# kohnakagawa/md_neighbor_list

Hardware: AMD Instinct MI355X
Metric: Verlet-list build ms and Mpairs/s at N=1M rho=1.0; achieved HBM GB/s (higher is better)
Workload: dtype f32

## Files before the change

md_neighbor_list_amd/csrc/nl_kernels.hpp:

```cpp
#pragma once

#include <hip/hip_runtime.h>
#include <stdint.h>

#include <type_traits>

namespace nl {

constexpr int WAVE = 64;

enum : uint32_t { ST_OUT_OF_BOX = 1u, ST_CAPACITY = 2u, ST_DOMAIN = 4u, ST_INDEX_OVERFLOW = 8u, ST_ROW_OVERFLOW = 16u };

template <typename T> struct Pos;
template <> struct alignas(16) Pos<float> {
  float x, y, z;
  int32_t gid;
};
template <> struct alignas(32) Pos<double> {
  double x, y, z;
  int32_t gid;
  int32_t row;
};

struct Box {
// ... 675 lines not shown
    const T t = mul_rn(q, ims);
    const T f = sub_rn(t, (T)(int32_t)t);
    return (f >= (T)0.25 ? 1 : 0) + (f >= (T)0.5 ? 1 : 0) + (f >= (T)0.75 ? 1 : 0);
  };
  const bool tilt = !FINE && IDC == 0 && g.tilt;
  auto bin_of = [&](const Pos<T>& p) {
    const int32_t c = tilt ? p.gid : xcell1(p.x);
    if constexpr (FINE) return quarter(p.z, g.ims[2]) * mx + c;
    else if constexpr (IDC > 0) return c * IDC + min((int32_t)((uint32_t)p.gid >> id_shift), IDC - 1);
    else return c;
  };
  constexpr int BC_KEEP = 6;
  const bool keep = end - beg <= BC_KEEP * 256 && end > beg && !(g.dbg & 512);
  Pos<T> pk[BC_KEEP];
  int32_t rk[BC_KEEP];
  if (keep) {
#pragma unroll
    for (int u = 0; u < BC_KEEP; u++) {
      const int32_t k = min(beg + tid + u * 256, end - 1);
      pk[u] = src[k];
      rk[u] = src_row[k];
    }
#pragma unroll
    for (int u = 0; u < BC_KEEP; u++) {
      keep_in_flight(pk[u].x), keep_in_flight(pk[u].y), keep_in_flight(pk[u].z), keep_in_flight(pk[u].gid), keep_in_flight(rk[u]);
      if constexpr (sizeof(T) == 8) keep_in_flight(pk[u].row);
    }
#pragma unroll
    for (int u = 0; u < BC_KEEP; u++)
      if (beg + tid + u * 256 < end) atomicAdd(&cnt[bin_of(pk[u])], 1);
  } else {
    for (int32_t k = beg + tid; k < end; k += 256) atomicAdd(&cnt[bin_of(src[k])], 1);
  }
  __syncthreads();
  for (int32_t base = 0; base < nb; base += 256) {
    const int32_t c = base + tid;
    const int32_t v = c < nb ? cnt[c] : 0;
    const int32_t inc = wave_incl_scan(v, lane);
    if (lane == 63) wsum[w] = inc;
    __syncthreads();
    int32_t woff = 0;
    for (int k = 0; k < w; k++) woff += wsum[k];
    const int32_t carry = carry_s;
    const int32_t excl = carry + woff + inc - v;
    if (c < nb) {
      cnt[c] = excl;
      if constexpr (FINE) {
        cell_start[((size_t)r * mx + (c % mx)) * 4 + c / mx] = beg + excl;
      } else if constexpr (IDC > 0) {
        cls_start[(size_t)r * nb + c] = beg + excl;
        if (c % IDC == 0) cell_start[(size_t)r * mx + c / IDC] = beg + excl;
      } else {
        cell_start[(size_t)r * nb + c] = beg + excl;
      }
    }
    __syncthreads();
    if (tid == 255) carry_s = carry + woff + inc;
    __syncthreads();
  }
  if (r == nrows - 1 && tid == 0) {
    if constexpr (IDC > 0) cls_start[(size_t)nrows * nb] = end, cell_start[(size_t)nrows * mx] = end;
    else cell_start[(size_t)nrows * nb] = end;
  }
  auto place = [&](Pos<T> p, int32_t row_of) {
    const int32_t dst = beg + atomicAdd(&cnt[bin_of(p)], 1);
    if (tilt) {
      p.gid = row_of;
    } else if (g.pbc & 1) {
      const T tx = mul_rn(p.x, g.ims[0]);
      int32_t v = (int32_t)tx;
      if (tx < (T)0 && (T)v != tx) v -= 1;
      if (v < 0) p.x = add_rn(p.x, g.L[0]);
      if (v >= mx) p.x = add_rn(p.x, -g.L[0]);
    }
    sorted[dst] = p;
    sorted_row[dst] = row_of;
    sorted_gid[dst] = p.gid;
  };
  if (keep) {
#pragma unroll
    for (int u = 0; u < BC_KEEP; u++)
      if (beg + tid + u * 256 < end) place(pk[u], rk[u]);
  } else {
    for (int32_t k = beg + tid; k < end; k += 256) place(src[k], src_row[k]);
  }
}

enum { MODE_COUNT = 0, MODE_FILL = 1, MODE_COUNT_MASKS = 2 };

struct FastDiv {
  uint32_t d, m, s;
};
__device__ __forceinline__ uint32_t fastdiv(uint32_t n, const FastDiv& f) {
  if (f.d == 1) return n;
  const uint32_t t = __umulhi(n, f.m);
  return (t + ((n - t) >> 1)) >> (f.s - 1);
}

template <typename T> struct SweepArgs {
  const Pos<T>* __restrict__ sorted;
  const int32_t* __restrict__ sorted_row;
  const int32_t* __restrict__ sorted_gid;
  const int32_t* __restrict__ cell_start;
  const int32_t* __restrict__ cls_start;
  int32_t mx, my, mzl, slab;
  FastDiv div_mx, div_my;
  T rc2;
  int32_t* __restrict__ count;
  int32_t* __restrict__ progress;
  const void* __restrict__ key_pointer;
  int32_t wide;
  int32_t n_rows;
  int32_t* __restrict__ list;
  const int64_t* __restrict__ total;
  int64_t capacity;
  uint32_t* __restrict__ status;
  T L[3];
  int32_t pbc;
  T ms[3];
  int32_t z_origin;
  int32_t isplit;
  int32_t mask_nb;
  int32_t* __restrict__ full27_list;
  int32_t* __restrict__ full27_count;
  int32_t* __restrict__ fill_list_count;
  uint32_t* __restrict__ masks;
  uint8_t* __restrict__ masks_hi;
  unsigned long long* dbg_buf;
  int32_t dbg;
  const uint32_t* gate = nullptr;
  T k[3];
  const double* lat;
};

template <typename T>
__device__ __forceinline__ void face_shift(const SweepArgs<T>& a, int32_t wr, T& sx, T& sy, T& sz) {
  T s[3];
  lattice_shift(a.lat, wr, s);
  sx = s[0], sy = s[1], sz = s[2];
}

__device__ __forceinline__ void recheck_image(const SweepArgs<double>& a, int32_t wr, Pos<double>& pe) {
  const double* p = a.lat + 3 * wr;
  pe.x = add_rn(pe.x, p[0]);
  __builtin_amdgcn_sched_barrier(0);
  pe.y = add_rn(pe.y, p[1]);
  __builtin_amdgcn_sched_barrier(0);
  pe.z = add_rn(pe.z, p[2]);
}

template <typename T> struct SweepCfg;
constexpr int MASK_LO_BYTES = 2 * WAVE, MASK_HI_BYTES = WAVE, MASK_ROW_BYTES = MASK_LO_BYTES + MASK_HI_BYTES;
__device__ __forceinline__ bool hi_plane_used(int32_t mask_nb, int32_t ntiles) { return mask_nb > 1 || ntiles > 16; }
template <bool NT = false>
__device__ __forceinline__ void mask_store(uint32_t* masks, uint8_t* masks_hi, size_t row, int lane, uint32_t bits, bool hi) {
  uint16_t* const lo_p = reinterpret_cast<uint16_t*>(reinterpret_cast<char*>(masks) + row * MASK_LO_BYTES) + lane;
  uint8_t* const hi_p = masks_hi + row * MASK_HI_BYTES + lane;
  if constexpr (NT) {
    __builtin_nontemporal_store((uint16_t)bits, lo_p);
    if (hi) __builtin_nontemporal_store((uint8_t)(bits >> 16), hi_p);
  } else {
    *lo_p = (uint16_t)bits;
    if (hi) *hi_p = (uint8_t)(bits >> 16);
  }
}
template <bool NT, typename P> __device__ __forceinline__ P mask_ld(const P* p) {
  if constexpr (NT) return __builtin_nontemporal_load(p);
  else return *p;
}
__device__ __forceinline__ uint32_t mask_load(const uint32_t* masks, const uint8_t* masks_hi, size_t row, int lane) {
  return (uint32_t)reinterpret_cast<const uint16_t*>(reinterpret_cast<const char*>(masks) + row * MASK_LO_BYTES)[lane] |
         (uint32_t)(masks_hi + row * MASK_HI_BYTES)[lane] << 16;
}
template <> struct SweepCfg<float> { static constexpr int CAP = 1280; };
template <> struct SweepCfg<double> { static constexpr int CAP = 1280; };

constexpr int SWEEP_WAVES = 4;
constexpr int SWEEP_G = 5;
constexpr int NSEG = 18;

struct alignas(16) PosS {
  float x, y, z;
  int32_t gid;
};
struct ScreenCtx {
  float lo, hi;
  float lo_in, hi_out;
  const int32_t* sidx;
  const uint8_t* swrap;
};
template <typename T, bool SCREEN> struct TileOf { typedef Pos<T> type; };
template <typename T> struct TileOf<T, true> { typedef PosS type; };

#ifndef NL_STAMP
#define NL_STAMP 0
#endif
#ifndef NL_STAMP_FILL
#define NL_STAMP_FILL 0
#endif
#ifndef NL_DIAG
#define NL_DIAG 0
#endif
constexpr int NL_PRIO = 3;
template <int GC>
__device__ __forceinline__ void r2_group_f32(float xj, float yj, float zj, const float* xi, const float* yi, const float* zi, float* r2) {
#pragma unroll
  for (int k = 0; k < GC; k++) {
    const float dx = sub_rn(xj, xi[k]), dy = sub_rn(yj, yi[k]), dz = sub_rn(zj, zi[k]);
    r2[k] = add_rn(add_rn(mul_rn(dx, dx), mul_rn(dy, dy)), mul_rn(dz, dz));
  }
}

template <typename T, int MODE, int GC, bool FULL = false, bool NOSELF = false, bool SCREEN = false, bool PBC = false>
__device__ __forceinline__ int32_t search_group(const SweepArgs<T>& a, const typename TileOf<T, SCREEN>::type* tile, int32_t nj,
                                                int32_t ntiles, int lane, const Pos<T>& pi_l, int64_t base_l,
                                                int32_t slot0 = 0, bool store_masks = false, int32_t self0 = 0, int32_t batch = 0,
                                                const ScreenCtx* sc = nullptr, float uxi_l = 0.f, float uyi_l = 0.f, float uzi_l = 0.f,
                                                uint32_t* words_out = nullptr) {
  static_assert(!NOSELF || (FULL && MODE == MODE_COUNT_MASKS), "NOSELF is a form of the full-list COUNT_MASKS search");
  static_assert(SweepCfg<T>::CAP / WAVE <= 24, "one bit per j-tile in the 24-bit word a lane keeps (mask_store)");
  static_assert(!SCREEN || sizeof(T) == 8, "the screened search is the fp64 search");
  typedef typename TileOf<T, SCREEN>::type TileT;
  typedef typename std::conditional<SCREEN, float, T>::type R;
  R xi[GC], yi[GC], zi[GC];
  int32_t gi[GC];
  uint32_t cur[GC];
  int32_t* rowp[GC];
  uint32_t bits[GC];
  constexpr bool VBITS_F32 = MODE == MODE_COUNT_MASKS && !SCREEN && sizeof(T) == 4 && (!FULL || NOSELF);
  constexpr bool VBITS_SCREEN = MODE == MODE_COUNT_MASKS && SCREEN && (!FULL || NOSELF);
  constexpr bool VBITS = VBITS_F32 || VBITS_SCREEN;
  uint32_t gi1[GC];
#pragma unroll
  for (int k = 0; k < GC; k++) bits[k] = 0;
#pragma unroll
  for (int k = 0; k < GC; k++) {
    if constexpr (SCREEN) {
      xi[k] = __builtin_bit_cast(float, __builtin_amdgcn_readlane(__builtin_bit_cast(int32_t, uxi_l), k));
      yi[k] = __builtin_bit_cast(float, __builtin_amdgcn_readlane(__builtin_bit_cast(int32_t, uyi_l), k));
      zi[k] = __builtin_bit_cast(float, __builtin_amdgcn_readlane(__builtin_bit_cast(int32_t, uzi_l), k));
    } else if constexpr (sizeof(T) == 4) {
      xi[k] = __builtin_bit_cast(float, __builtin_amdgcn_readlane(__builtin_bit_cast(int32_t, pi_l.x), k));
      yi[k] = __builtin_bit_cast(float, __builtin_amdgcn_readlane(__builtin_bit_cast(int32_t, pi_l.y), k));
      zi[k] = __builtin_bit_cast(float, __builtin_amdgcn_readlane(__builtin_bit_cast(int32_t, pi_l.z), k));
    } else {
      xi[k] = __shfl(pi_l.x, k, WAVE);
      yi[k] = __shfl(pi_l.y, k, WAVE);
      zi[k] = __shfl(pi_l.z, k, WAVE);
    }
    gi[k] = __builtin_amdgcn_readlane(pi_l.gid, k);
    cur[k] = 0u;
    gi1[k] = (uint32_t)gi[k] + 1u;
    if (MODE == MODE_FILL) {
      const uint32_t lo = (uint32_t)__builtin_amdgcn_readlane((int32_t)(uint32_t)base_l, k);
      const uint32_t hi = (uint32_t)__builtin_amdgcn_readlane((int32_t)(uint32_t)((uint64_t)base_l >> 32), k);
      rowp[k] = a.list + (int64_t)(((uint64_t)hi << 32) | lo);
    }
  }

  auto test_tile = [&](const TileT& pj, int32_t tix) {
    if constexpr (VBITS_SCREEN) {
      constexpr int HALF = (GC + 1) / 2;
      uint32_t uacc = 0;
#pragma unroll
      for (int k = 0; k < GC; k++) {
        if (k == HALF) __builtin_amdgcn_sched_barrier(0);
        const float dx = pj.x - xi[k], dy = pj.y - yi[k], dz = pj.z - zi[k];
        const float r2 = __builtin_fmaf(dz, dz, __builtin_fmaf(dy, dy, dx * dx));
        const uint32_t t_in = __builtin_bit_cast(uint32_t, sc->lo_in - r2), t_out = __builtin_bit_cast(uint32_t, r2 - sc->hi_out);
        uint32_t w = t_in;
        if (!NOSELF) w |= (uint32_t)pj.gid - gi1[k];
        bits[k] = __builtin_amdgcn_alignbit(bits[k], w, 31);
        uacc |= t_in & t_out;
      }
      if (__builtin_amdgcn_ballot_w64((int32_t)uacc < 0) != 0) {
        const int32_t at = tix * WAVE + lane;
        Pos<double> pe;
        pe.x = 0, pe.y = 0, pe.z = 0;
        if ((int32_t)uacc < 0) {
          pe = a.sorted[sc->sidx[at]];
          if (PBC) recheck_image(a, sc->swrap[at], pe);
        }
#pragma unroll
        for (int k = 0; k < GC; k++) {
          const float dx = pj.x - xi[k], dy = pj.y - yi[k], dz = pj.z - zi[k];
          const float r2 = __builtin_fmaf(dz, dz, __builtin_fmaf(dy, dy, dx * dx));
          const bool unc = (int32_t)(__builtin_bit_cast(uint32_t, sc->lo_in - r2) & __builtin_bit_cast(uint32_t, r2 - sc->hi_out)) < 0;
          if (__builtin_amdgcn_ballot_w64(unc) == 0) continue;
          const double xe = __hiloint2double(__builtin_amdgcn_readlane(__double2hiint(pi_l.x), k), __builtin_amdgcn_readlane(__double2loint(pi_l.x), k));
          const double ye = __hiloint2double(__builtin_amdgcn_readlane(__double2hiint(pi_l.y), k), __builtin_amdgcn_readlane(__double2loint(pi_l.y), k));
          const double ze = __hiloint2double(__builtin_amdgcn_readlane(__double2hiint(pi_l.z), k), __builtin_amdgcn_readlane(__double2loint(pi_l.z), k));
          const double ex = sub_rn(pe.x, xe), ey = sub_rn(pe.y, ye), ez = sub_rn(pe.z, ze);
          const double e2 = add_rn(add_rn(mul_rn(ex, ex), mul_rn(ey, ey)), mul_rn(ez, ez));
          const bool upper = NOSELF ? true : pj.gid > gi[k];
          if (unc && !(e2 > a.rc2) && upper) bits[k] &= ~1u;
        }
      }
      return;
    }
    if constexpr (VBITS_F32) {
      constexpr int HALF = (GC + 1) / 2;
#pragma unroll
      for (int k = 0; k < GC; k++) {
        if (k == HALF) __builtin_amdgcn_sched_barrier(0);
        const float dx = sub_rn(pj.x, xi[k]), dy = sub_rn(pj.y, yi[k]), dz = sub_rn(pj.z, zi[k]);
        const float r2 = add_rn(add_rn(mul_rn(dx, dx), mul_rn(dy, dy)), mul_rn(dz, dz));
// ... 453 lines not shown
  }
#endif
}

template <typename T, int MODE> constexpr int sweep_cap() { return SweepCfg<T>::CAP; }

template <typename T, int MODE, bool FULL = false, bool PBC = false>
__device__ __forceinline__ void sweep_cell(const SweepArgs<T>& a) {
  if (gate_closed(a.gate)) return;
  constexpr int CAP = sweep_cap<T, MODE>();
  constexpr bool SCREEN = sizeof(T) == 8;
  __shared__ __attribute__((aligned(32))) char tile_bytes[SCREEN ? screen_lds_bytes(CAP) : CAP * (int)sizeof(Pos<T>)];
  Pos<T>* const tile = reinterpret_cast<Pos<T>*>(tile_bytes);
  if (MODE == MODE_FILL) {
    if (a.total[0] > a.capacity) {
      if (blockIdx.x == 0 && threadIdx.x == 0) atomicOr(a.status, ST_CAPACITY);
      return;
    }
  }
  const int tid = threadIdx.x, lane = tid & 63, wave = __builtin_amdgcn_readfirstlane(tid >> 6);
  CellCtx c;
  if (MODE == MODE_COUNT_MASKS) __builtin_amdgcn_s_setprio(NL_PRIO);
#if NL_STAMP
  const uint64_t t_entry = __builtin_amdgcn_s_memtime();
#endif
  if (MODE == MODE_COUNT_MASKS || a.isplit <= 1) {
    if (!cell_setup(a, lane, c)) return;
  } else {
    const int32_t wp = xcd_cell_index(), w = wp / a.isplit, part = wp - w * a.isplit;
    const int32_t wy = (int32_t)fastdiv((uint32_t)w, a.div_mx), cx = w - wy * a.mx;
    const int32_t wz = (int32_t)fastdiv((uint32_t)wy, a.div_my), cy = wy - wz * a.my, cz = wz + (a.slab ? 1 : 0);
    if (!cell_setup_at(a, lane, cx, cy, cz, c)) return;
    const int32_t lo = (int32_t)((int64_t)c.ni * part / a.isplit), hi = (int32_t)((int64_t)c.ni * (part + 1) / a.isplit);
    c.ibeg += lo, c.ni = hi - lo;
    if (c.ni <= 0) return;
  }
#if NL_STAMP
  if (MODE == MODE_COUNT_MASKS && lane == 0) atomicAdd(a.dbg_buf + 64 + (blockIdx.x & 1023) * 16, (unsigned long long)(__builtin_amdgcn_s_memtime() - t_entry));
#endif
  cell_search<T, MODE, CAP, SWEEP_WAVES, FULL, PBC, SCREEN>(a, c, tile, tid, lane, wave);
}

template <typename T, int MODE, bool FULL = false, bool PBC = false>
__global__ void __launch_bounds__(SWEEP_WAVES* WAVE) k_sweep(SweepArgs<T> a) {
  sweep_cell<T, MODE, FULL, PBC>(a);
}
template <bool FULL = false, bool PBC = false>
__global__ void __launch_bounds__(SWEEP_WAVES* WAVE) __attribute__((amdgpu_num_sgpr(80)))
k_sweep_count_f32(SweepArgs<float> a) {
  sweep_cell<float, MODE_COUNT, FULL, PBC>(a);
}
template <bool FULL = false, bool PBC = false>
__global__ void __launch_bounds__(SWEEP_WAVES* WAVE) __attribute__((amdgpu_num_sgpr(80)))
k_sweep_count_masks_f32(SweepArgs<float> a) {
  sweep_cell<float, MODE_COUNT_MASKS, FULL, PBC>(a);
}

__device__ __forceinline__ int32_t scan64_dpp(int32_t v) {
  v += __builtin_amdgcn_update_dpp(0, v, 0x111, 0xf, 0xf, false);
  v += __builtin_amdgcn_update_dpp(0, v, 0x112, 0xf, 0xf, false);
  v += __builtin_amdgcn_update_dpp(0, v, 0x114, 0xf, 0xf, false);
  v += __builtin_amdgcn_update_dpp(0, v, 0x118, 0xf, 0xf, false);
  v += __builtin_amdgcn_update_dpp(0, v, 0x142, 0xa, 0xf, false);
  v += __builtin_amdgcn_update_dpp(0, v, 0x143, 0xc, 0xf, false);
  return v;
}

constexpr int CLS_OWN = 13;
template <int IDC> struct ClsCtx {
  static constexpr int NWIN = 27 * IDC, NT = (NWIN + WAVE - 1) / WAVE;
  int32_t ibeg, ni, total_j;
  int32_t cx, cy, cz;
  int32_t src[NT], len[NT], off[NT];
  __device__ __forceinline__ int32_t get(const int32_t (&v)[NT], int32_t w) const {
    if constexpr (NT == 1) return __builtin_amdgcn_readlane(v[0], w);
    else return w < WAVE ? __builtin_amdgcn_readlane(v[0], w) : __builtin_amdgcn_readlane(v[1], w - WAVE);
  }
};

template <int IDC>
__device__ __forceinline__ bool cls_setup_at(const SweepArgs<float>& a, int lane, int32_t cx, int32_t cy, int32_t cz, ClsCtx<IDC>& c) {
  typedef ClsCtx<IDC> X;
  const int32_t cell = cx + (cy + cz * a.my) * a.mx;
  const uint32_t st_word = *a.status;
  c.ibeg = a.cell_start[cell];
  c.ni = a.cell_start[cell + 1] - c.ibeg;
  c.cx = cx, c.cy = cy, c.cz = cz;
#pragma unroll
  for (int j = 0; j < X::NT; j++) {
    const int32_t w = j * WAVE + lane;
    int32_t src = 0, len = 0;
    if (w < X::NWIN) {
      const int32_t k = w / 27, s = w - 27 * k, r9 = s / 3;
      int32_t x = cx + (s - 3 * r9) - 1, y = cy + r9 % 3 - 1, z = cz + r9 / 3 - 1;
      x += x < 0 ? a.mx : x >= a.mx ? -a.mx : 0;
      y += y < 0 ? a.my : y >= a.my ? -a.my : 0;
      z += z < 0 ? a.mzl : z >= a.mzl ? -a.mzl : 0;
      const int32_t e = (x + (y + z * a.my) * a.mx) * IDC + k;
      src = a.cls_start[e];
      len = a.cls_start[e + 1] - src;
    }
    c.src[j] = src, c.len[j] = len;
  }
  if (c.ni <= 0 || (st_word & ST_DOMAIN)) return false;
  int32_t carry = 0;
#pragma unroll
  for (int j = 0; j < X::NT; j++) {
    const int32_t incl = scan64_dpp(c.len[j]);
    c.off[j] = carry + incl - c.len[j];
    carry += __builtin_amdgcn_readlane(incl, 63);
  }
  c.total_j = carry;
  return true;
}
template <int IDC> __device__ __forceinline__ bool cls_setup(const SweepArgs<float>& a, int lane, ClsCtx<IDC>& c) {
  const int32_t w = xcd_cell_index();
  const int32_t wy = (int32_t)fastdiv((uint32_t)w, a.div_mx), cx = w - wy * a.mx;
  const int32_t cz = (int32_t)fastdiv((uint32_t)wy, a.div_my), cy = wy - cz * a.my;
  return cls_setup_at(a, lane, cx, cy, cz, c);
}

template <int IDC, int NW, typename E>
__device__ __forceinline__ void cls_stage(const E* __restrict__ from, const ClsCtx<IDC>& c, E* dst, int lane, int wave) {
#pragma unroll 1
  for (int32_t pc = wave; pc < 9 * IDC; pc += NW) {
    const int32_t w = 3 * pc;
    const int32_t s0 = c.get(c.src, w), l0 = c.get(c.len, w), s1 = c.get(c.src, w + 1), l1 = c.get(c.len, w + 1);
    const int32_t s2 = c.get(c.src, w + 2), l2 = c.get(c.len, w + 2), off = c.get(c.off, w);
    const int32_t len = l0 + l1 + l2;
#pragma unroll 1
    for (int32_t kb = 0; kb < len; kb += WAVE) {
      const int32_t i = kb + lane;
      if (i < len) {
        const int32_t at = i < l0 ? s0 + i : i < l0 + l1 ? s1 + (i - l0) : s2 + (i - l0 - l1);
        const __attribute__((address_space(1))) void* const gp = (const __attribute__((address_space(1))) void*)(from + at);
        __attribute__((address_space(3))) void* const lp = (__attribute__((address_space(3))) void*)(dst + off + kb);
        if constexpr (sizeof(E) == 16) __builtin_amdgcn_global_load_lds(gp, lp, 16, 0, 0);
        else __builtin_amdgcn_global_load_lds(gp, lp, 4, 0, 0);
      }
    }
  }
}

template <bool FULL> constexpr int EXPAND_RMAX_OF = FULL ? 192 : 160;
constexpr int EXPAND_WAVES = 2;

template <typename T, bool FULL = false, bool PBC = false, typename OFF = int32_t, int RB = 24, int EW = EXPAND_WAVES, int CAP = SweepCfg<T>::CAP,
          int IDC = 0>
__global__ void __launch_bounds__(EW* WAVE, (sizeof(OFF) == 8 ? 4 : sizeof(T) == 4 ? (FULL || RB > 12 ? 7 : 8) : 4)) __attribute__((amdgpu_num_sgpr(80)))
k_fill_masks(SweepArgs<T> a) {
  static_assert(IDC == 0 || (sizeof(T) == 4 && !FULL && !PBC), "id classes: fp32 half list, open box");
  if (gate_closed(a.gate)) return;
  constexpr int EXPAND_RMAX = EXPAND_RMAX_OF<FULL>;
  __shared__ __attribute__((aligned(32))) int32_t lds[CAP + EW * 4 * EXPAND_RMAX];
  int32_t* const gids = lds;
  const int tid = threadIdx.x, lane = tid & 63, wave = __builtin_amdgcn_readfirstlane(tid >> 6);
#if NL_STAMP_FILL
  uint64_t ft_prev = __builtin_amdgcn_s_memtime(), ft_acc[6] = {0, 0, 0, 0, 0, 0};
  auto fstamp = [&](int phase) {
    const uint64_t now = __builtin_amdgcn_s_memtime();
    ft_acc[phase] += now - ft_prev;
    ft_prev = now;
  };
#endif
  const int64_t total = a.total[0];
  typename std::conditional<(IDC > 0), ClsCtx<IDC ? IDC : 2>, CellCtx>::type c;
  bool ok;
  if constexpr (IDC > 0) ok = cls_setup<IDC>(a, lane, c);
  else ok = cell_setup(a, lane, c);
#if NL_STAMP_FILL
  fstamp(0);
#endif
  if (total > a.capacity) {
    if (blockIdx.x == 0 && threadIdx.x == 0) atomicOr(a.status, ST_CAPACITY);
    return;
  }
  if (!ok) return;
  if (c.total_j > CAP) {
    if (tid == 0) a.full27_list[atomicAdd(a.fill_list_count, 1)] = c.cx + (c.cy + c.cz * a.my) * a.mx;
    return;
  }

  const int32_t per_wave = (c.ni + EW - 1) / EW;
  const int32_t r_beg = min(wave * per_wave, c.ni), r_end = min(r_beg + per_wave, c.ni);
  uint32_t w[RB];
  OFF base_l;
  const bool hi_plane = hi_plane_used(1, (c.total_j + WAVE - 1) / WAVE);
  auto load_rows = [&](int32_t r0) {
    {
      const int32_t srow = a.sorted_row[c.ibeg + r0 + min(lane, RB - 1)];
      base_l = static_cast<const OFF*>(a.key_pointer)[min((uint32_t)srow, (uint32_t)a.n_rows)];
    }
    const size_t slot0 = (size_t)(c.ibeg + r0);
    const char* const lo0 = reinterpret_cast<const char*>(a.masks) + slot0 * MASK_LO_BYTES;
    if (hi_plane) {
      const uint8_t* const hi0 = a.masks_hi + slot0 * MASK_HI_BYTES;
#pragma unroll
      for (int u = 0; u < RB; u++)
        w[u] = (uint32_t)mask_ld<EW == 2>(reinterpret_cast<const uint16_t*>(lo0 + u * MASK_LO_BYTES) + lane) | (uint32_t)mask_ld<EW == 2>(hi0 + u * MASK_HI_BYTES + lane) << 16;
    } else {
#pragma unroll
      for (int u = 0; u < RB; u++) w[u] = (uint32_t)mask_ld<EW == 2>(reinterpret_cast<const uint16_t*>(lo0 + u * MASK_LO_BYTES) + lane);
    }
  };
  auto base = [&](int u) -> OFF {
    const uint32_t lo = (uint32_t)__builtin_amdgcn_readlane((int32_t)(uint32_t)base_l, u);
    if constexpr (sizeof(OFF) == 4) return (OFF)lo;
    const uint32_t hi = (uint32_t)__builtin_amdgcn_readlane((int32_t)(uint32_t)((uint64_t)base_l >> 32), u);
    return (OFF)((uint64_t)hi << 32 | lo);
  };
  load_rows(r_beg);
  if (a.dbg & 32) return;

  int32_t cls_row[IDC > 0 ? IDC : 1], cls_t0[IDC > 0 ? IDC : 1];
  if constexpr (IDC > 0) {
#pragma unroll
    for (int k = 0; k < IDC; k++) {
      cls_row[k] = c.get(c.src, 27 * k + CLS_OWN) - c.ibeg;
      cls_t0[k] = c.get(c.off, 27 * k) & ~(WAVE - 1);
    }
    cls_stage<IDC, EW>(a.sorted_gid, c, gids, lane, wave);
  } else
#pragma unroll
  for (int s = 0; s < (NSEG + EW - 1) / EW; s++) {
    const int sg = min(wave + s * EW, NSEG - 1);
    const int32_t len = wave + s * EW < NSEG ? __builtin_amdgcn_readlane(c.seg_len, sg) : 0;
    const int32_t src = __builtin_amdgcn_readlane(c.seg_src, sg);
    const int32_t off = __builtin_amdgcn_readlane(c.seg_off, sg);
    for (int32_t kb = 0; kb < len; kb += WAVE) {
      if (kb + lane < len)
        __builtin_amdgcn_global_load_lds((const __attribute__((address_space(1))) void*)(a.sorted_gid + src + kb + lane),
                                         (__attribute__((address_space(3))) void*)(gids + off + kb), 4, 0, 0);
    }
  }
#if NL_STAMP_FILL
  fstamp(1);
#endif
  __syncthreads();
#if NL_STAMP_FILL
  fstamp(2);
#endif

  const int32_t* const g = gids + lane;
  for (int32_t r0 = r_beg; r0 < r_end; r0 += RB) {
    if (r0 != r_beg) load_rows(r0);
#pragma unroll
    for (int u0 = 0; u0 < RB; u0 += 4) {
      if (r0 + u0 >= r_end) continue;
      uint32_t word[4], ptr[4];
      int32_t nrow[4];
      const int32_t* gq[4];
#pragma unroll
      for (int q = 0; q < 4; q++) {
        if constexpr (IDC > 0) {
          int32_t t0 = cls_t0[0];
#pragma unroll
          for (int k = 1; k < IDC; k++) t0 = r0 + u0 + q >= cls_row[k] ? cls_t0[k] : t0;
          gq[q] = g + t0;
        } else {
          gq[q] = g;
        }
      }
#pragma unroll
      for (int q = 0; q < 4; q++) {
        word[q] = r0 + u0 + q < r_end ? (w[u0 + q] & 0xFFFFFFu) : 0u;
        if (a.dbg & 16) word[q] = 0;
        const int32_t cnt = __popc(word[q]);
        const int32_t incl = scan64_dpp(cnt);
        nrow[q] = __builtin_amdgcn_readlane(incl, 63);
        ptr[q] = (uint32_t)(incl - cnt);
      }
      const int32_t nmax = max(max(nrow[0], nrow[1]), max(nrow[2], nrow[3]));
#if NL_STAMP_FILL
      fstamp(3);
#endif
      if (nmax <= EXPAND_RMAX) {
        int32_t* const cw = lds + CAP + wave * 4 * EXPAND_RMAX;
#pragma unroll
        for (int q = 0; q < 4; q++) ptr[q] += q * EXPAND_RMAX;
        while (word[0] | word[1] | word[2] | word[3]) {
          int32_t val[4];
          bool on[4];
#pragma unroll
          for (int q = 0; q < 4; q++) {
            on[q] = word[q] != 0;
            const int32_t t = on[q] ? __ffs(word[q]) - 1 : 0;
            val[q] = gq[q][t * WAVE];
          }
#pragma unroll
          for (int q = 0; q < 4; q++) {
            if (on[q]) {
              cw[ptr[q]] = val[q];
              ptr[q]++;
              word[q] &= word[q] - 1;
            }
          }
        }
#if NL_STAMP_FILL
        fstamp(4);
#endif
        __builtin_amdgcn_wave_barrier();
        for (int32_t e = lane; e - lane < nmax; e += WAVE) {
          int32_t val[4];
#pragma unroll
          for (int q = 0; q < 4; q++) val[q] = cw[q * EXPAND_RMAX + min(e, EXPAND_RMAX - 1)];
#pragma unroll
          for (int q = 0; q < 4; q++)
            if (e < nrow[q]) a.list[(size_t)base(u0 + q) + e] = val[q];
        }
        __builtin_amdgcn_wave_barrier();
#if NL_STAMP_FILL
        fstamp(5);
#endif
        continue;
      }
      while (word[0] | word[1] | word[2] | word[3]) {
        int32_t val[4];
        bool on[4];
#pragma unroll
        for (int q = 0; q < 4; q++) {
          on[q] = word[q] != 0;
          const int32_t t = on[q] ? __ffs(word[q]) - 1 : 0;
          val[q] = gq[q][t * WAVE];
        }
#pragma unroll
        for (int q = 0; q < 4; q++) {
          if (on[q]) {
            a.list[(size_t)base(u0 + q) + ptr[q]] = val[q];
            ptr[q]++;
            word[q] &= word[q] - 1;
          }
        }
      }
    }
  }
#if NL_STAMP_FILL
  if (lane == 0) {
    unsigned long long* const slot = a.dbg_buf + 64 + (blockIdx.x & 1023) * 16;
    for (int ph = 0; ph < 6; ph++) atomicAdd(slot + ph, (unsigned long long)ft_acc[ph]);
    atomicAdd(slot + 9, 1ull);
  }
#endif
}

template <typename T, bool FULL = false, bool PBC = false>
__global__ void __launch_bounds__(SWEEP_WAVES* WAVE) k_fill_list(SweepArgs<T> a) {
  if (gate_closed(a.gate)) return;
  constexpr int CAP = sweep_cap<T, MODE_FILL>();
  constexpr bool SCREEN = sizeof(T) == 8;
  __shared__ __attribute__((aligned(32))) char tile_bytes[SCREEN ? screen_lds_bytes(CAP) : CAP * (int)sizeof(Pos<T>)];
  Pos<T>* const tile = reinterpret_cast<Pos<T>*>(tile_bytes);
  if (a.total[0] > a.capacity) return;
  const int tid = threadIdx.x, lane = tid & 63, wave = __builtin_amdgcn_readfirstlane(tid >> 6);
  const int32_t count = *a.fill_list_count;
  for (int32_t idx = blockIdx.x; idx < count; idx += gridDim.x) {
    if (idx != (int32_t)blockIdx.x) __syncthreads();
    const int32_t cell = a.full27_list[idx];
    const int32_t row = cell / a.mx, cx = cell - row * a.mx, cz = row / a.my, cy = row - cz * a.my;
    CellCtx c;
    if (!cell_setup_at(a, lane, cx, cy, cz, c)) continue;
    cell_search<T, MODE_FILL, CAP, SWEEP_WAVES, FULL, PBC, SCREEN>(a, c, tile, tid, lane, wave);
  }
}

constexpr int FD_NB = 7;
constexpr int FD_WAVES = 4;
constexpr int FD_RMAX = 1024;

template <typename T, bool FULL = false, bool PBC = false, typename OFF = int32_t>
__global__ void __launch_bounds__(FD_WAVES* WAVE) k_fill_dense(SweepArgs<T> a, const OFF* __restrict__ base_sorted) {
  if (gate_closed(a.gate)) return;
  constexpr int CAP = SweepCfg<T>::CAP;
  __shared__ __attribute__((aligned(32))) int32_t lds[FD_NB * CAP + FD_WAVES * FD_RMAX];
  int32_t* const gids = lds;
  const int tid = threadIdx.x, lane = tid & 63, wave = __builtin_amdgcn_readfirstlane(tid >> 6);
  const int64_t total = a.total[0];
  CellCtx c;
  const bool ok = cell_setup(a, lane, c);
  if (total > a.capacity) {
    if (blockIdx.x == 0 && threadIdx.x == 0) atomicOr(a.status, ST_CAPACITY);
    return;
  }
  if (!ok) return;
  const int32_t nbatch = (c.total_j + CAP - 1) / CAP;
  if (nbatch > a.mask_nb) {
    constexpr int CAPS = (int)(FD_NB * CAP * sizeof(int32_t) / sizeof(Pos<T>)) / WAVE * WAVE;
    cell_search<T, MODE_FILL, CAPS, FD_WAVES, FULL, PBC>(a, c, reinterpret_cast<Pos<T>*>(gids), tid, lane, wave);
    return;
  }
  const int32_t nb = a.mask_nb;
  constexpr int FD_RB = 4;
  auto load_rows = [&](int32_t r0, uint32_t (&w)[FD_RB][FD_NB], OFF (&base)[FD_RB]) {
#pragma unroll
    for (int u = 0; u < FD_RB; u++) {
      const int32_t slot = c.ibeg + min(r0 + u * FD_WAVES, c.ni - 1);
      base[u] = base_sorted[slot];
#pragma unroll
      for (int b = 0; b < FD_NB; b++) w[u][b] = mask_load(a.masks, a.masks_hi, (size_t)slot * nb + min(b, nb - 1), lane);
    }
#pragma unroll
    for (int u = 0; u < FD_RB; u++)
#pragma unroll
      for (int b = 0; b < FD_NB; b++) asm volatile("" : "+v"(w[u][b]));
#pragma unroll
    for (int u = 0; u < FD_RB; u++)
#pragma unroll
      for (int b = 0; b < FD_NB; b++) w[u][b] = (b < nbatch && r0 + u * FD_WAVES < c.ni) ? (w[u][b] & 0xFFFFFFu) : 0u;
  };
  uint32_t wb[FD_RB][FD_NB];
  OFF baseb[FD_RB];
  for (int32_t sg = wave; sg < NSEG; sg += FD_WAVES) {
    const int32_t len = __builtin_amdgcn_readlane(c.seg_len, sg);
    const int32_t src = __builtin_amdgcn_readlane(c.seg_src, sg);
    const int32_t off = __builtin_amdgcn_readlane(c.seg_off, sg);
    for (int32_t kb = 0; kb < len; kb += WAVE) {
      if (kb + lane < len)
        __builtin_amdgcn_global_load_lds((const __attribute__((address_space(1))) void*)(a.sorted_gid + src + kb + lane),
                                         (__attribute__((address_space(3))) void*)(gids + off + kb), 4, 0, 0);
    }
  }
  __syncthreads();
  const int32_t* const g = gids + lane;
  int32_t* const cw = lds + FD_NB * CAP + wave * FD_RMAX;
  for (int32_t rb = wave; rb < c.ni; rb += FD_WAVES * FD_RB) {
    load_rows(rb, wb, baseb);
#pragma unroll
    for (int u = 0; u < FD_RB; u++) {
    const int32_t r = rb + u * FD_WAVES;
    if (r >= c.ni) break;
    uint32_t (&wd)[FD_NB] = wb[u];
    const OFF base = baseb[u];
    int32_t cnt = 0;
#pragma unroll
    for (int b = 0; b < FD_NB; b++) cnt += __popc(wd[b]);
    const int32_t incl = scan64_dpp(cnt);
    const int32_t nrow = __builtin_amdgcn_readlane(incl, 63);
    uint32_t ptr = (uint32_t)(incl - cnt);
    const bool in_lds = nrow <= FD_RMAX;
#pragma unroll
    for (int b = 0; b < FD_NB; b += 2) {
      if (b >= nbatch) break;
      uint32_t w0 = wd[b], w1 = b + 1 < FD_NB ? wd[b + 1] : 0u;
      const int32_t* const g0 = g + b * CAP;
      const int32_t* const g1 = g + (b + 1 < FD_NB ? b + 1 : b) * CAP;
      uint32_t p0 = ptr, p1 = ptr + (uint32_t)__popc(w0);
      ptr = p1 + (uint32_t)__popc(w1);
      while (__builtin_amdgcn_ballot_w64((w0 | w1) != 0)) {
        const bool on0 = w0 != 0, on1 = w1 != 0;
        const int32_t v0 = g0[(on0 ? __ffs(w0) - 1 : 0) * WAVE];
        const int32_t v1 = g1[(on1 ? __ffs(w1) - 1 : 0) * WAVE];
        if (on0) {
          if (in_lds) cw[p0] = v0;
          else a.list[(size_t)base + p0] = v0;
          p0++, w0 &= w0 - 1;
        }
        if (on1) {
          if (in_lds) cw[p1] = v1;
          else a.list[(size_t)base + p1] = v1;
          p1++, w1 &= w1 - 1;
        }
      }
    }
    if (in_lds) {
      __builtin_amdgcn_wave_barrier();
      for (int32_t e = lane; e < nrow; e += WAVE) a.list[(size_t)base + e] = cw[e];
      __builtin_amdgcn_wave_barrier();
    }
    }
  }
}

}

#include "nl_lean.hpp"
#include "nl_rows.hpp"

namespace nl {

template <typename OFF>
__global__ void __launch_bounds__(256) k_row_base(const OFF* __restrict__ key_pointer,
                                                   const int32_t* __restrict__ sorted_row, int32_t n_rows, int32_t n,
                                                   OFF* __restrict__ base_sorted, const uint32_t* __restrict__ gate = nullptr) {
  if (gate_closed(gate)) return;
  const int32_t s = blockIdx.x * blockDim.x + threadIdx.x;
  if (s >= n) return;
  const int32_t r = sorted_row[s];
  base_sorted[s] = (uint32_t)r < (uint32_t)n_rows ? key_pointer[r] : (OFF)0;
}

}
```

md_neighbor_list_amd/csrc/nl_lean.hpp:

```cpp
#pragma once

namespace nl {

constexpr int PIPE_G = 7;

template <int NW = SWEEP_WAVES>
__device__ __forceinline__ void pipe_stage(const SweepArgs<float>& a, const CellCtx& c, Pos<float>* dst, int tid, int lane, int wave) {
#pragma unroll 1
  for (int sg = wave; sg < NSEG; sg += NW) {
    const int32_t len = __builtin_amdgcn_readlane(c.seg_len, sg);
    const int32_t src = __builtin_amdgcn_readlane(c.seg_src, sg);
    const int32_t off = __builtin_amdgcn_readlane(c.seg_off, sg);
#pragma unroll 1
    for (int32_t kb = 0; kb < len; kb += WAVE) {
      if (kb + lane < len)
        __builtin_amdgcn_global_load_lds((const __attribute__((address_space(1))) void*)(a.sorted + src + kb + lane),
                                         (__attribute__((address_space(3))) void*)(dst + off + kb), 16, 0, 0);
    }
  }
  const int32_t pad = c.total_j + tid;
  if (pad < ((c.total_j + WAVE - 1) & ~(WAVE - 1))) {
    Pos<float> sentinel;
    sentinel.x = 1.0e18f, sentinel.y = 0.f, sentinel.z = 0.f, sentinel.gid = INT32_MIN;
    dst[pad] = sentinel;
// ... 13 lines not shown
  for (int k = 0; k < PIPE_G; k++)
    if (k < p.gcount) mask_store<NT>(a.masks, a.masks_hi, (size_t)(p.slot0 + k) * a.mask_nb, lane, p.w[k], hi);
  p.gcount = 0;
}

template <bool FULL, int GC>
__device__ __forceinline__ void pipe_group(const SweepArgs<float>& a, const Pos<float>* tile, int32_t nj, int32_t ntiles, int lane,
                                           const Pos<float>& pi_l, int32_t slot0, int32_t self0, PipePending& p) {
  uint32_t words[GC];
  p.mine = search_group<float, MODE_COUNT_MASKS, GC, FULL, FULL, false, false>(a, tile, nj, ntiles, lane, pi_l, 0, slot0, true, self0,
                                                                             0, nullptr, 0.f, 0.f, 0.f, words);
#pragma unroll
  for (int k = 0; k < GC; k++) p.w[k] = words[k];
}

template <bool FULL, int NW = SWEEP_WAVES>
__device__ __forceinline__ void pipe_search(const SweepArgs<float>& a, const CellCtx& c, const Pos<float>* tile, int lane, int wave,
                                            PipePending& p) {
  constexpr int G = PIPE_G;
  const int32_t ibeg = c.ibeg, ni = c.ni, nj = c.total_j;
  const int32_t ntiles = (nj + WAVE - 1) / WAVE;
  const int32_t rounds = (ni + NW * G - 1) / (NW * G);
  const int32_t ngroups = rounds * NW;
  const int32_t gbase = ni / ngroups, grem = ni - gbase * ngroups;
  const int32_t s4 = __builtin_amdgcn_readlane(c.seg_src, 4), l4 = __builtin_amdgcn_readlane(c.seg_len, 4);
  const bool in4 = ibeg >= s4 && ibeg < s4 + l4;
  const int32_t own = in4 ? __builtin_amdgcn_readlane(c.seg_off, 4) + ibeg - s4
                          : __builtin_amdgcn_readlane(c.seg_off, 13) + ibeg - __builtin_amdgcn_readlane(c.seg_src, 13);
  for (int32_t g = wave; g < ngroups; g += NW) {
    const int32_t i0 = g * gbase + min(g, grem);
    const int32_t gcount = gbase + (g < grem ? 1 : 0);
    if (gcount <= 0) break;
    pipe_flush<NW == SWEEP_WAVES>(a, p, lane, hi_plane_used(a.mask_nb, ntiles));
    const int32_t k = min(lane, gcount - 1);
    Pos<float> pi_l = tile[own + i0 + k];
    const int32_t row_l = a.sorted_row[ibeg + i0 + k];
    if (lane >= gcount) pi_l.x = 0, pi_l.y = 0, pi_l.z = 0, pi_l.gid = 0;
    const int32_t slot0 = ibeg + i0, self0 = own + i0;
    switch (gcount) {
      case 1: pipe_group<FULL, 1>(a, tile, nj, ntiles, lane, pi_l, slot0, self0, p); break;
      case 2: pipe_group<FULL, 2>(a, tile, nj, ntiles, lane, pi_l, slot0, self0, p); break;
      case 3: pipe_group<FULL, 3>(a, tile, nj, ntiles, lane, pi_l, slot0, self0, p); break;
      case 4: pipe_group<FULL, 4>(a, tile, nj, ntiles, lane, pi_l, slot0, self0, p); break;
      case 5: pipe_group<FULL, 5>(a, tile, nj, ntiles, lane, pi_l, slot0, self0, p); break;
      case 6: pipe_group<FULL, 6>(a, tile, nj, ntiles, lane, pi_l, slot0, self0, p); break;
      default: pipe_group<FULL, 7>(a, tile, nj, ntiles, lane, pi_l, slot0, self0, p); break;
    }
    p.row_l = row_l, p.slot0 = slot0, p.gcount = gcount;
  }
}

constexpr int LEAN_SMALL_CAP = SweepCfg<float>::CAP / 2;
template <bool FULL, int NW = SWEEP_WAVES, int CAP = SweepCfg<float>::CAP>
__global__ void __launch_bounds__(NW* WAVE, 8) __attribute__((amdgpu_num_sgpr(80))) k_sweep_lean_f32(SweepArgs<float> a) {
  if (gate_closed(a.gate)) return;
  __shared__ __attribute__((aligned(32))) Pos<float> buf[CAP];
  const int tid = threadIdx.x, lane = tid & 63, wave = __builtin_amdgcn_readfirstlane(tid >> 6);
  __builtin_amdgcn_s_setprio(NL_PRIO);
  CellCtx c;
  if (!cell_setup(a, lane, c)) return;
  if (c.total_j > CAP) {
    if (tid == 0) a.full27_list[atomicAdd(a.full27_count, 1)] = c.cx + (c.cy + c.cz * a.my) * a.mx;
    return;
  }
  pipe_stage<NW>(a, c, buf, tid, lane, wave);
  asm volatile("s_waitcnt vmcnt(0) lgkmcnt(0)\n\ts_barrier" ::: "memory");
  PipePending pend;
  pend.gcount = 0, pend.mine = 0, pend.row_l = 0, pend.slot0 = 0;
  pipe_search<FULL, NW>(a, c, buf, lane, wave, pend);
  pipe_flush<NW == SWEEP_WAVES>(a, pend, lane, hi_plane_used(a.mask_nb, (c.total_j + WAVE - 1) / WAVE));
}

template <int GC>
__device__ __forceinline__ int32_t class_group(const SweepArgs<float>& a, const Pos<float>* tile, int32_t t0, int32_t tsplit,
                                               int32_t ntiles, int lane, const Pos<float>& pi_l, uint32_t* words) {
  float xi[GC], yi[GC], zi[GC];
  uint32_t gi1[GC], bits[GC];
#pragma unroll
  for (int k = 0; k < GC; k++) {
    xi[k] = __builtin_bit_cast(float, __builtin_amdgcn_readlane(__builtin_bit_cast(int32_t, pi_l.x), k));
    yi[k] = __builtin_bit_cast(float, __builtin_amdgcn_readlane(__builtin_bit_cast(int32_t, pi_l.y), k));
    zi[k] = __builtin_bit_cast(float, __builtin_amdgcn_readlane(__builtin_bit_cast(int32_t, pi_l.z), k));
    gi1[k] = (uint32_t)__builtin_amdgcn_readlane(pi_l.gid, k) + 1u;
    bits[k] = 0;
  }
  auto test_tile = [&](const Pos<float>& pj, auto id) {
    constexpr int HALF = (GC + 1) / 2;
#pragma unroll
    for (int k = 0; k < GC; k++) {
      if (k == HALF) __builtin_amdgcn_sched_barrier(0);
      const float dx = sub_rn(pj.x, xi[k]), dy = sub_rn(pj.y, yi[k]), dz = sub_rn(pj.z, zi[k]);
      const float r2 = add_rn(add_rn(mul_rn(dx, dx), mul_rn(dy, dy)), mul_rn(dz, dz));
      uint32_t w = __builtin_bit_cast(uint32_t, sub_rn(a.rc2, r2));
      if constexpr (decltype(id)::value) w |= (uint32_t)pj.gid - gi1[k];
      bits[k] = __builtin_amdgcn_alignbit(bits[k], w, 31);
    }
  };
  const std::true_type with_id;
  const std::false_type no_id;
  const int32_t last = (ntiles - 1) * WAVE + lane;
  Pos<float> pa = tile[t0 * WAVE + lane], pb;
  int32_t t = t0;
  __builtin_amdgcn_s_setprio(0);
  for (; t + 1 < tsplit; t += 2) {
    pb = tile[(t + 1) * WAVE + lane];
    test_tile(pa, with_id);
    pa = tile[min((t + 2) * WAVE + lane, last)];
    test_tile(pb, with_id);
  }
  if (t < tsplit) {
    test_tile(pa, with_id);
    t++;
    pa = tile[min(t * WAVE + lane, last)];
  }
  for (; t + 1 < ntiles; t += 2) {
    pb = tile[(t + 1) * WAVE + lane];
    test_tile(pa, no_id);
    pa = tile[min((t + 2) * WAVE + lane, last)];
    test_tile(pb, no_id);
  }
  if (t < ntiles) test_tile(pa, no_id);
  __builtin_amdgcn_s_setprio(NL_PRIO);
  const int32_t nt = ntiles - t0;
  uint32_t tot[GC];
#pragma unroll
  for (int k = 0; k < GC; k++) words[k] = __brev(~bits[k]) >> (32 - nt);
#pragma unroll
  for (int k = 0; k < GC; k += 2) {
    const uint32_t two = wave_sum_dpp((uint32_t)__popc(words[k]) | (k + 1 < GC ? (uint32_t)__popc(words[k + 1]) << 16 : 0u));
    tot[k] = two & 0xffffu;
    if (k + 1 < GC) tot[k + 1] = two >> 16;
  }
  uint32_t mine = 0;
#pragma unroll
  for (int k = 0; k < GC; k++) mine = lane == k ? tot[k] : mine;
  return (int32_t)mine;
}

template <int GC>
__device__ __forceinline__ void class_pipe_group(const SweepArgs<float>& a, const Pos<float>* tile, int32_t t0, int32_t tsplit,
                                                 int32_t ntiles, int lane, const Pos<float>& pi_l, PipePending& p) {
  uint32_t words[GC];
  p.mine = class_group<GC>(a, tile, t0, tsplit, ntiles, lane, pi_l, words);
#pragma unroll
  for (int k = 0; k < GC; k++) p.w[k] = words[k];
}

template <int IDC, int NW>
__device__ __forceinline__ void class_search(const SweepArgs<float>& a, const ClsCtx<IDC>& c, const Pos<float>* tile, int lane, int wave,
                                             PipePending& p) {
  constexpr int G = PIPE_G, NP = IDC / 2, WP = NW / NP;
  static_assert(NW % NP == 0, "waves a pair of classes");
  const int32_t ntiles = (c.total_j + WAVE - 1) / WAVE;
  const bool hi = hi_plane_used(1, ntiles);
  const int pair = wave / WP, wj = wave - pair * WP;
#pragma unroll
  for (int h = 0; h < 2; h++) {
    const int32_t k = h == 0 ? pair : IDC - 1 - pair;
    const int32_t ni = c.get(c.len, 27 * k + CLS_OWN);
    const int32_t own = c.get(c.off, 27 * k + CLS_OWN), slot_b = c.get(c.src, 27 * k + CLS_OWN);
    const int32_t t0 = c.get(c.off, 27 * k) / WAVE;
    const int32_t tsplit = k + 1 < IDC ? (c.get(c.off, 27 * (k + 1)) + WAVE - 1) / WAVE : ntiles;
    const int32_t ngroups = (ni + WP * G - 1) / (WP * G) * WP;
    if (ni <= 0) continue;
    const int32_t gbase = ni / ngroups, grem = ni - gbase * ngroups;
    for (int32_t g = wj; g < ngroups; g += WP) {
      const int32_t i0 = g * gbase + min(g, grem);
      const int32_t gcount = gbase + (g < grem ? 1 : 0);
      if (gcount <= 0) break;
      pipe_flush<NW == SWEEP_WAVES>(a, p, lane, hi);
      const int32_t kk = min(lane, gcount - 1);
      Pos<float> pi_l = tile[own + i0 + kk];
      const int32_t row_l = a.sorted_row[slot_b + i0 + kk];
      if (lane >= gcount) pi_l.x = 0, pi_l.y = 0, pi_l.z = 0, pi_l.gid = 0;
      switch (gcount) {
        case 1: class_pipe_group<1>(a, tile, t0, tsplit, ntiles, lane, pi_l, p); break;
        case 2: class_pipe_group<2>(a, tile, t0, tsplit, ntiles, lane, pi_l, p); break;
        case 3: class_pipe_group<3>(a, tile, t0, tsplit, ntiles, lane, pi_l, p); break;
        case 4: class_pipe_group<4>(a, tile, t0, tsplit, ntiles, lane, pi_l, p); break;
        case 5: class_pipe_group<5>(a, tile, t0, tsplit, ntiles, lane, pi_l, p); break;
        case 6: class_pipe_group<6>(a, tile, t0, tsplit, ntiles, lane, pi_l, p); break;
        default: class_pipe_group<7>(a, tile, t0, tsplit, ntiles, lane, pi_l, p); break;
      }
      p.row_l = row_l, p.slot0 = slot_b + i0, p.gcount = gcount;
    }
  }
}

template <int IDC, int NW = SWEEP_WAVES, int CAP = SweepCfg<float>::CAP>
__global__ void __launch_bounds__(NW* WAVE, 8) __attribute__((amdgpu_num_sgpr(80))) k_sweep_class_f32(SweepArgs<float> a) {
  if (gate_closed(a.gate)) return;
  __shared__ __attribute__((aligned(32))) Pos<float> buf[CAP];
  const int tid = threadIdx.x, lane = tid & 63, wave = __builtin_amdgcn_readfirstlane(tid >> 6);
  __builtin_amdgcn_s_setprio(NL_PRIO);
  ClsCtx<IDC> c;
  if (!cls_setup<IDC>(a, lane, c)) return;
  if (c.total_j > CAP) {
    if (tid == 0) a.full27_list[atomicAdd(a.full27_count, 1)] = c.cx + (c.cy + c.cz * a.my) * a.mx;
    return;
  }
  cls_stage<IDC, NW>(a.sorted, c, buf, lane, wave);
  const int32_t pad = c.total_j + tid;
  if (pad < ((c.total_j + WAVE - 1) & ~(WAVE - 1))) {
    Pos<float> sentinel;
    sentinel.x = 1.0e18f, sentinel.y = 0.f, sentinel.z = 0.f, sentinel.gid = INT32_MIN;
    buf[pad] = sentinel;
  }
  asm volatile("s_waitcnt vmcnt(0) lgkmcnt(0)\n\ts_barrier" ::: "memory");
  PipePending pend;
  pend.gcount = 0, pend.mine = 0, pend.row_l = 0, pend.slot0 = 0;
  class_search<IDC, NW>(a, c, buf, lane, wave, pend);
  pipe_flush<NW == SWEEP_WAVES>(a, pend, lane, hi_plane_used(1, (c.total_j + WAVE - 1) / WAVE));
}

template <bool FULL>
__global__ void __launch_bounds__(SWEEP_WAVES* WAVE) __attribute__((amdgpu_num_sgpr(80))) k_sweep_list_f32(SweepArgs<float> a) {
  if (gate_closed(a.gate)) return;
  constexpr int CAP = SweepCfg<float>::CAP;
  __shared__ __attribute__((aligned(32))) Pos<float> tile[CAP];
  const int tid = threadIdx.x, lane = tid & 63, wave = __builtin_amdgcn_readfirstlane(tid >> 6);
  const int32_t count = *a.full27_count;
  for (int32_t idx = blockIdx.x; idx < count; idx += gridDim.x) {
    if (idx != (int32_t)blockIdx.x) __syncthreads();
    const int32_t cell = a.full27_list[idx];
    const int32_t row = cell / a.mx, cx = cell - row * a.mx, cz = row / a.my, cy = row - cz * a.my;
    CellCtx c;
    if (!cell_setup_at(a, lane, cx, cy, cz, c)) continue;
    cell_search<float, MODE_COUNT_MASKS, CAP, SWEEP_WAVES, FULL, false, false>(a, c, tile, tid, lane, wave);
  }
}

}
```

Before: 160,700.

## Deal id-class rows across waves and skip unused high mask plane per class

Decides per id class whether the high 8-bit mask plane is needed, based on that class's tile span, so both the sweep writer and the fill reader skip hi-plane traffic when a class fits in 16 tiles. In the fill kernel with two classes, each wave now takes half of each class's rows, so every wave loads rows from both classes. Pairs of popcount scans are packed into one 16+16-bit DPP scan, and the expand loop uses a branchless scatter to a dummy LDS slot. The group split for the second class is mirrored so short groups fall at the other end. Writer and reader must agree on the per-class hi decision; the packed counts limit rows to 65535 pairs.

```diff
diff --git a/md_neighbor_list_amd/csrc/nl_kernels.hpp b/md_neighbor_list_amd/csrc/nl_kernels.hpp
--- a/md_neighbor_list_amd/csrc/nl_kernels.hpp
+++ b/md_neighbor_list_amd/csrc/nl_kernels.hpp
@@ -851,6 +851,7 @@
 template <typename T> struct SweepCfg;
 constexpr int MASK_LO_BYTES = 2 * WAVE, MASK_HI_BYTES = WAVE, MASK_ROW_BYTES = MASK_LO_BYTES + MASK_HI_BYTES;
 __device__ __forceinline__ bool hi_plane_used(int32_t mask_nb, int32_t ntiles) { return mask_nb > 1 || ntiles > 16; }
+__device__ __forceinline__ bool cls_hi_plane(int32_t ntiles, int32_t t0) { return ntiles - t0 > 16; }
 template <bool NT = false>
 __device__ __forceinline__ void mask_store(uint32_t* masks, uint8_t* masks_hi, size_t row, int lane, uint32_t bits, bool hi) {
   uint16_t* const lo_p = reinterpret_cast<uint16_t*>(reinterpret_cast<char*>(masks) + row * MASK_LO_BYTES) + lane;
@@ -1610,7 +1611,8 @@
   static_assert(IDC == 0 || (sizeof(T) == 4 && !FULL && !PBC), "id classes: fp32 half list, open box");
   if (gate_closed(a.gate)) return;
   constexpr int EXPAND_RMAX = EXPAND_RMAX_OF<FULL>;
-  __shared__ __attribute__((aligned(32))) int32_t lds[CAP + EW * 4 * EXPAND_RMAX];
+  constexpr bool DEAL = IDC == 2 && RB == 24 && EW == 2;
+  __shared__ __attribute__((aligned(32))) int32_t lds[CAP + EW * 4 * EXPAND_RMAX + (DEAL ? EW * WAVE : 0)];
   int32_t* const gids = lds;
   const int tid = threadIdx.x, lane = tid & 63, wave = __builtin_amdgcn_readfirstlane(tid >> 6);
 #if NL_STAMP_FILL
@@ -1639,19 +1641,59 @@
     return;
   }
 
+  int32_t cls_row[IDC > 0 ? IDC : 1], cls_t0[IDC > 0 ? IDC : 1];
+  bool cls_hi[IDC > 0 ? IDC : 1];
+  if constexpr (IDC > 0) {
+#pragma unroll
+    for (int k = 0; k < IDC; k++) {
+      cls_row[k] = c.get(c.src, 27 * k + CLS_OWN) - c.ibeg;
+      cls_t0[k] = c.get(c.off, 27 * k) & ~(WAVE - 1);
+      cls_hi[k] = cls_hi_plane((c.total_j + WAVE - 1) / WAVE, cls_t0[k] / WAVE);
+    }
+  }
+  constexpr int RH = RB / 2;
   const int32_t per_wave = (c.ni + EW - 1) / EW;
   const int32_t r_beg = min(wave * per_wave, c.ni), r_end = min(r_beg + per_wave, c.ni);
+  int32_t ch_beg[2] = {0, 0}, ch_end[2] = {0, 0};
+  if constexpr (DEAL) {
+    const int32_t n0 = cls_row[1], n1 = c.ni - n0;
+    int32_t s0 = min(n0, (((n0 + 1) >> 1) + 3) & ~3), s1 = (n1 >> 1) & ~3;
+    if (n1 - s1 > RH && n1 <= 2 * RH) s1 = n1 - RH;
+    ch_beg[0] = wave ? s0 : 0, ch_end[0] = wave ? n0 : s0;
+    ch_beg[1] = n0 + (wave ? s1 : 0), ch_end[1] = n0 + (wave ? n1 : s1);
+  }
   uint32_t w[RB];
   OFF base_l;
-  const bool hi_plane = hi_plane_used(1, (c.total_j + WAVE - 1) / WAVE);
-  auto load_rows = [&](int32_t r0) {
+  bool hi_plane;
+  if constexpr (IDC > 0) hi_plane = cls_hi[0];
+  else hi_plane = hi_plane_used(1, (c.total_j + WAVE - 1) / WAVE);
+  auto load_rows = [&](int32_t r0, int32_t rb) {
     {
-      const int32_t srow = a.sorted_row[c.ibeg + r0 + min(lane, RB - 1)];
+      int32_t slot = c.ibeg + r0 + min(lane, RB - 1);
+      if constexpr (DEAL) slot = c.ibeg + (lane < RH ? r0 + lane : rb + min(lane, RB - 1) - RH);
+      const int32_t srow = a.sorted_row[slot];
       base_l = static_cast<const OFF*>(a.key_pointer)[min((uint32_t)srow, (uint32_t)a.n_rows)];
     }
     const size_t slot0 = (size_t)(c.ibeg + r0);
     const char* const lo0 = reinterpret_cast<const char*>(a.masks) + slot0 * MASK_LO_BYTES;
-    if (hi_plane) {
+    if constexpr (DEAL) {
+      const uint8_t* const hi0 = a.masks_hi + slot0 * MASK_HI_BYTES;
+      const size_t slot1 = (size_t)(c.ibeg + rb);
+      const char* const lo1 = reinterpret_cast<const char*>(a.masks) + slot1 * MASK_LO_BYTES;
+      const uint8_t* const hi1 = a.masks_hi + slot1 * MASK_HI_BYTES;
+      auto lo_of = [&](int u) { return (uint32_t)mask_ld<true>(reinterpret_cast<const uint16_t*>((u < RH ? lo0 : lo1) + (u % RH) * MASK_LO_BYTES) + lane); };
+      auto hi_of = [&](int u) { return (uint32_t)mask_ld<true>((u < RH ? hi0 : hi1) + (u % RH) * MASK_HI_BYTES + lane) << 16; };
+      if (cls_hi[1]) {
+#pragma unroll
+        for (int u = 0; u < RB; u++) w[u] = lo_of(u) | hi_of(u);
+      } else if (cls_hi[0]) {
+#pragma unroll
+        for (int u = 0; u < RB; u++) w[u] = u < RH ? lo_of(u) | hi_of(u) : lo_of(u);
+      } else {
+#pragma unroll
+        for (int u = 0; u < RB; u++) w[u] = lo_of(u);
+      }
+    } else if (hi_plane) {
       const uint8_t* const hi0 = a.masks_hi + slot0 * MASK_HI_BYTES;
 #pragma unroll
       for (int u = 0; u < RB; u++)
@@ -1667,16 +1709,10 @@
     const uint32_t hi = (uint32_t)__builtin_amdgcn_readlane((int32_t)(uint32_t)((uint64_t)base_l >> 32), u);
     return (OFF)((uint64_t)hi << 32 | lo);
   };
-  load_rows(r_beg);
+  load_rows(DEAL ? ch_beg[0] : r_beg, ch_beg[1]);
   if (a.dbg & 32) return;
 
-  int32_t cls_row[IDC > 0 ? IDC : 1], cls_t0[IDC > 0 ? IDC : 1];
   if constexpr (IDC > 0) {
-#pragma unroll
-    for (int k = 0; k < IDC; k++) {
-      cls_row[k] = c.get(c.src, 27 * k + CLS_OWN) - c.ibeg;
-      cls_t0[k] = c.get(c.off, 27 * k) & ~(WAVE - 1);
-    }
     cls_stage<IDC, EW>(a.sorted_gid, c, gids, lane, wave);
   } else
 #pragma unroll
@@ -1700,33 +1736,64 @@
 #endif
 
   const int32_t* const g = gids + lane;
-  for (int32_t r0 = r_beg; r0 < r_end; r0 += RB) {
-    if (r0 != r_beg) load_rows(r0);
+  for (int32_t r0 = DEAL ? ch_beg[0] : r_beg, rb = ch_beg[1], done = 0; DEAL || r0 < r_end; r0 += RB, done += RH) {
+    if constexpr (DEAL) {
+      r0 = min(ch_beg[0] + done, ch_end[0]), rb = min(ch_beg[1] + done, ch_end[1]);
+      if (r0 >= ch_end[0] && rb >= ch_end[1]) break;
+      if (done) load_rows(r0, rb);
+    } else {
+      if (r0 != r_beg) load_rows(r0, 0);
+    }
 #pragma unroll
     for (int u0 = 0; u0 < RB; u0 += 4) {
-      if (r0 + u0 >= r_end) continue;
+      int32_t row0 = r0 + u0, rend = r_end;
+      if constexpr (DEAL) row0 = u0 < RH ? r0 + u0 : rb + (u0 - RH), rend = ch_end[u0 < RH ? 0 : 1];
+      if (row0 >= rend) continue;
       uint32_t word[4], ptr[4];
       int32_t nrow[4];
       const int32_t* gq[4];
+      uint32_t wmask[4];
 #pragma unroll
       for (int q = 0; q < 4; q++) {
-        if constexpr (IDC > 0) {
+        wmask[q] = 0xFFFFFFu;
+        if constexpr (DEAL) {
+          gq[q] = g + cls_t0[u0 < RH ? 0 : 1];
+        } else if constexpr (IDC > 0) {
           int32_t t0 = cls_t0[0];
-#pragma unroll
-          for (int k = 1; k < IDC; k++) t0 = r0 + u0 + q >= cls_row[k] ? cls_t0[k] : t0;
+          bool hi = cls_hi[0];
+#pragma unroll
+          for (int k = 1; k < IDC; k++) {
+            const bool up = row0 + q >= cls_row[k];
+            t0 = up ? cls_t0[k] : t0;
+            hi = up ? cls_hi[k] : hi;
+          }
           gq[q] = g + t0;
+          wmask[q] = hi ? 0xFFFFFFu : 0xFFFFu;
         } else {
           gq[q] = g;
         }
       }
 #pragma unroll
       for (int q = 0; q < 4; q++) {
-        word[q] = r0 + u0 + q < r_end ? (w[u0 + q] & 0xFFFFFFu) : 0u;
+        word[q] = row0 + q < rend ? (w[u0 + q] & 0xFFFFFFu) : 0u;
+        if constexpr (IDC > 0 && !DEAL) word[q] &= wmask[q];
         if (a.dbg & 16) word[q] = 0;
-        const int32_t cnt = __popc(word[q]);
-        const int32_t incl = scan64_dpp(cnt);
-        nrow[q] = __builtin_amdgcn_readlane(incl, 63);
-        ptr[q] = (uint32_t)(incl - cnt);
+        if constexpr (!DEAL) {
+          const int32_t cnt = __popc(word[q]);
+          const int32_t incl = scan64_dpp(cnt);
+          nrow[q] = __builtin_amdgcn_readlane(incl, 63);
+          ptr[q] = (uint32_t)(incl - cnt);
+        }
+      }
+      if constexpr (DEAL) {
+#pragma unroll
+        for (int q = 0; q < 4; q += 2) {
+          const int32_t c0 = __popc(word[q]), c1 = __popc(word[q + 1]);
+          const uint32_t incl = (uint32_t)scan64_dpp(c0 | c1 << 16);
+          const uint32_t tot = (uint32_t)__builtin_amdgcn_readlane((int32_t)incl, 63);
+          nrow[q] = (int32_t)(tot & 0xffffu), nrow[q + 1] = (int32_t)(tot >> 16);
+          ptr[q] = (incl & 0xffffu) - (uint32_t)c0, ptr[q + 1] = (incl >> 16) - (uint32_t)c1;
+        }
       }
       const int32_t nmax = max(max(nrow[0], nrow[1]), max(nrow[2], nrow[3]));
 #if NL_STAMP_FILL
@@ -1736,6 +1803,7 @@
         int32_t* const cw = lds + CAP + wave * 4 * EXPAND_RMAX;
 #pragma unroll
         for (int q = 0; q < 4; q++) ptr[q] += q * EXPAND_RMAX;
+        const uint32_t nowhere = (uint32_t)((EW - wave) * 4 * EXPAND_RMAX + wave * WAVE + lane);
         while (word[0] | word[1] | word[2] | word[3]) {
           int32_t val[4];
           bool on[4];
@@ -1747,7 +1815,11 @@
           }
 #pragma unroll
           for (int q = 0; q < 4; q++) {
-            if (on[q]) {
+            if constexpr (DEAL) {
+              cw[on[q] ? ptr[q] : nowhere] = val[q];
+              ptr[q] += on[q] ? 1u : 0u;
+              word[q] &= word[q] - 1;
+            } else if (on[q]) {
               cw[ptr[q]] = val[q];
               ptr[q]++;
               word[q] &= word[q] - 1;
@@ -1794,9 +1866,9 @@
   }
 #if NL_STAMP_FILL
   if (lane == 0) {
-    unsigned long long* const slot = a.dbg_buf + 64 + (blockIdx.x & 1023) * 16;
+    unsigned long long* const slot = a.dbg_buf + 64 + (blockIdx.x & 1023) * 16 + 8 * wave;
     for (int ph = 0; ph < 6; ph++) atomicAdd(slot + ph, (unsigned long long)ft_acc[ph]);
-    atomicAdd(slot + 9, 1ull);
+    atomicAdd(slot + 6, 1ull);
   }
 #endif
 }
diff --git a/md_neighbor_list_amd/csrc/nl_lean.hpp b/md_neighbor_list_amd/csrc/nl_lean.hpp
--- a/md_neighbor_list_amd/csrc/nl_lean.hpp
+++ b/md_neighbor_list_amd/csrc/nl_lean.hpp
@@ -189,7 +189,7 @@
   constexpr int G = PIPE_G, NP = IDC / 2, WP = NW / NP;
   static_assert(NW % NP == 0, "waves a pair of classes");
   const int32_t ntiles = (c.total_j + WAVE - 1) / WAVE;
-  const bool hi = hi_plane_used(1, ntiles);
+  bool hi = false;
   const int pair = wave / WP, wj = wave - pair * WP;
 #pragma unroll
   for (int h = 0; h < 2; h++) {
@@ -201,11 +201,13 @@
     const int32_t ngroups = (ni + WP * G - 1) / (WP * G) * WP;
     if (ni <= 0) continue;
     const int32_t gbase = ni / ngroups, grem = ni - gbase * ngroups;
+    const int32_t gfirst = h == 0 ? 0 : ngroups - grem;
     for (int32_t g = wj; g < ngroups; g += WP) {
-      const int32_t i0 = g * gbase + min(g, grem);
-      const int32_t gcount = gbase + (g < grem ? 1 : 0);
-      if (gcount <= 0) break;
+      const int32_t i0 = g * gbase + (h == 0 ? min(g, grem) : max(g - gfirst, 0));
+      const int32_t gcount = gbase + (g >= gfirst && g < gfirst + grem ? 1 : 0);
+      if (gcount <= 0) continue;
       pipe_flush<NW == SWEEP_WAVES>(a, p, lane, hi);
+      hi = cls_hi_plane(ntiles, t0);
       const int32_t kk = min(lane, gcount - 1);
       Pos<float> pi_l = tile[own + i0 + kk];
       const int32_t row_l = a.sorted_row[slot_b + i0 + kk];
@@ -222,6 +224,7 @@
       p.row_l = row_l, p.slot0 = slot_b + i0, p.gcount = gcount;
     }
   }
+  pipe_flush<NW == SWEEP_WAVES>(a, p, lane, hi);
 }
 
 template <int IDC, int NW = SWEEP_WAVES, int CAP = SweepCfg<float>::CAP>
@@ -247,7 +250,6 @@
   PipePending pend;
   pend.gcount = 0, pend.mine = 0, pend.row_l = 0, pend.slot0 = 0;
   class_search<IDC, NW>(a, c, buf, lane, wave, pend);
-  pipe_flush<NW == SWEEP_WAVES>(a, pend, lane, hi_plane_used(1, (c.total_j + WAVE - 1) / WAVE));
 }
 
 template <bool FULL>
```

New measurement: 159,800. Within noise of the previous version (-0.6%).
